# yahoo/CaffeOnSpark

Hardware: NVIDIA H100
Metric: images/sec (higher is better)
Workload: dtype f32

## Files before the change

### caffeonspark_b200/csrc/caffe_layers.cu

```cuda
#include <math.h>

#include "caffe_layers.hpp"

namespace cosb {
namespace {

struct FastDiv {
  unsigned d, m, s;
  explicit FastDiv(unsigned div) : d(div), m(0), s(0) {
    while (s < 31 && (1u << s) < d) ++s;
    m = (unsigned)((((1ull << 32) * ((1ull << s) - d)) / d) + 1);
  }
  __device__ __forceinline__ unsigned div(unsigned n) const { return (__umulhi(n, m) + n) >> s; }
};

constexpr int kLrnChunk = 16;
constexpr int kLrnBlock = 128;

template <int HALF>
__global__ void __launch_bounds__(kLrnBlock) lrn_forward_kernel(const float* __restrict__ x, float* __restrict__ y,
                                                                int C, FastDiv fd_hw, unsigned npix, int nchunks,
                                                                float alpha_over_n, float beta, float k) {
  const int chunk = blockIdx.x % nchunks;
  const unsigned p = (blockIdx.x / nchunks) * kLrnBlock + threadIdx.x;
  if (p >= npix) return;
  const unsigned HW = fd_hw.d, n = fd_hw.div(p);
  const size_t base = (size_t)n * C * HW + (p - n * HW);
  const int c0 = chunk * kLrnChunk;
  float xv[kLrnChunk + 2 * HALF];
#pragma unroll
  for (int i = 0; i < kLrnChunk + 2 * HALF; ++i) {
    const int c = c0 - HALF + i;
    xv[i] = (c >= 0 && c < C) ? x[base + (size_t)c * HW] : 0.f;
  }
#pragma unroll
  for (int t = 0; t < kLrnChunk; ++t) {
    const int c = c0 + t;
    if (c < C) {
      float ss = 0.f;
#pragma unroll
      for (int j = 0; j <= 2 * HALF; ++j) ss += xv[t + j] * xv[t + j];
      const float s = k + alpha_over_n * ss;
      y[base + (size_t)c * HW] = xv[t + HALF] * powf(s, -beta);
    }
  }
}

template <int HALF>
__global__ void __launch_bounds__(kLrnBlock) lrn_backward_kernel(const float* __restrict__ x,
                                                                 const float* __restrict__ dy, float* __restrict__ dx,
                                                                 int C, FastDiv fd_hw, unsigned npix, int nchunks,
                                                                 float alpha_over_n, float beta, float k, float coef) {
  const int chunk = blockIdx.x % nchunks;
  const unsigned p = (blockIdx.x / nchunks) * kLrnBlock + threadIdx.x;
  if (p >= npix) return;
  const unsigned HW = fd_hw.d, n = fd_hw.div(p);
  const size_t base = (size_t)n * C * HW + (p - n * HW);
  const int c0 = chunk * kLrnChunk;
  constexpr int NR = kLrnChunk + 2 * HALF;
  float xv[NR + 2 * HALF];
  float dv[NR];
#pragma unroll
  for (int i = 0; i < NR + 2 * HALF; ++i) {
    const int c = c0 - 2 * HALF + i;
    xv[i] = (c >= 0 && c < C) ? x[base + (size_t)c * HW] : 0.f;
  }
#pragma unroll
  for (int i = 0; i < NR; ++i) {
    const int c = c0 - HALF + i;
    dv[i] = (c >= 0 && c < C) ? dy[base + (size_t)c * HW] : 0.f;
  }
  float r[NR], sb[NR];
#pragma unroll
  for (int i = 0; i < NR; ++i) {
    const int c = c0 - HALF + i;
    float ss = 0.f;
#pragma unroll
    for (int j = 0; j <= 2 * HALF; ++j) ss += xv[i + j] * xv[i + j];
    const float s = k + alpha_over_n * ss;
    sb[i] = powf(s, -beta);
    r[i] = (c >= 0 && c < C) ? dv[i] * xv[i + HALF] * sb[i] / s : 0.f;
  }
#pragma unroll
  for (int t = 0; t < kLrnChunk; ++t) {
    const int c = c0 + t;
    if (c < C) {
      float acc = 0.f;
#pragma unroll
      for (int j = 0; j <= 2 * HALF; ++j) acc += r[t + j];
      dx[base + (size_t)c * HW] = dv[t + HALF] * sb[t + HALF] - coef * xv[t + 2 * HALF] * acc;
    }
  }
}

template <template <int> class Launch, typename... A>
cudaError_t lrn_dispatch(int half, A... args) {
  switch (half) {
    case 0: return Launch<0>::run(args...);
    case 1: return Launch<1>::run(args...);
    case 2: return Launch<2>::run(args...);
    case 3: return Launch<3>::run(args...);
    case 4: return Launch<4>::run(args...);
    case 5: return Launch<5>::run(args...);
    case 6: return Launch<6>::run(args...);
    case 7: return Launch<7>::run(args...);
  }
  return cudaErrorInvalidValue;
}

struct LrnGrid {
  long long npix;
  int nchunks;
  long long blocks;
  FastDiv fd_hw;
  LrnGrid(int num, int channels, int hw)
      : npix((long long)num * hw), nchunks((channels + kLrnChunk - 1) / kLrnChunk),
        blocks(((npix + kLrnBlock - 1) / kLrnBlock) * nchunks), fd_hw(hw) {}
  bool fits() const { return npix < (1ll << 31) && blocks < (1ll << 31); }
};

template <int HALF>
struct LrnFwd {
  static cudaError_t run(const float* x, float* y, int C, const LrnGrid& g, float aon, float beta, float k,
                         cudaStream_t st) {
    lrn_forward_kernel<HALF><<<(unsigned)g.blocks, kLrnBlock, 0, st>>>(x, y, C, g.fd_hw, (unsigned)g.npix,
                                                                        g.nchunks, aon, beta, k);
    return cudaGetLastError();
  }
};

template <int HALF>
struct LrnBwd {
  static cudaError_t run(const float* x, const float* dy, float* dx, int C, const LrnGrid& g, float aon, float beta,
                         float k, float coef, cudaStream_t st) {
    lrn_backward_kernel<HALF><<<(unsigned)g.blocks, kLrnBlock, 0, st>>>(x, dy, dx, C, g.fd_hw, (unsigned)g.npix,
                                                                         g.nchunks, aon, beta, k, coef);
    return cudaGetLastError();
  }
};


template <int KERNEL, int STRIDE>
__global__ void pool_forward_kernel(const float* __restrict__ x, const float* __restrict__ bias,
                                    float* __restrict__ y, uint8_t* __restrict__ index, unsigned total, FastDiv fd_pp,
                                    FastDiv fd_pw, FastDiv fd_c, int H, int W, int kernel_rt, int stride_rt) {
  const int kernel = KERNEL ? KERNEL : kernel_rt, stride = STRIDE ? STRIDE : stride_rt;
  const unsigned i = blockIdx.x * blockDim.x + threadIdx.x;
  if (i >= total) return;
  const unsigned plane = fd_pp.div(i);
  const unsigned e = i - plane * fd_pp.d;
  const int ph = (int)fd_pw.div(e);
  const int pw = (int)(e - ph * fd_pw.d);
  const float b = bias[plane - fd_c.div(plane) * fd_c.d];
  const float* xp = x + (size_t)plane * H * W;
  const int hs = ph * stride, ws = pw * stride;
  float vmax = -INFINITY;
  int pos = 0;
#pragma unroll
  for (int dh = 0; dh < (KERNEL ? KERNEL : 15); ++dh) {
    if (dh >= kernel || hs + dh >= H) break;
#pragma unroll
    for (int dw = 0; dw < (KERNEL ? KERNEL : 15); ++dw) {
      if (dw >= kernel || ws + dw >= W) break;
      const float v = xp[(hs + dh) * W + ws + dw] + b;
      if (v > vmax || isnan(v)) {
        vmax = v;
        pos = dh * kernel + dw;
      }
    }
  }
  const bool pass = vmax > 0.f || isnan(vmax);
  y[i] = pass ? vmax : 0.f;
  index[i] = pass ? (uint8_t)pos : kPoolNoGrad;
}

template <int KERNEL, int STRIDE>
__global__ void pool_backward_kernel(const float* __restrict__ dy, const uint8_t* __restrict__ index,
                                     float* __restrict__ dx, float* __restrict__ partials, FastDiv fd_w, int H,
                                     int kernel_rt, int stride_rt, int PH, int PW) {
  const int kernel = KERNEL ? KERNEL : kernel_rt, stride = STRIDE ? STRIDE : stride_rt;
  const int W = (int)fd_w.d;
  const long long plane = blockIdx.x;
  const float* dyp = dy + (size_t)plane * PH * PW;
  const uint8_t* ip = index + (size_t)plane * PH * PW;
  float* dxp = dx + (size_t)plane * H * W;
  float part = 0.f;
  for (int e = threadIdx.x; e < H * W; e += blockDim.x) {
    const int h = (int)fd_w.div(e), w = e - h * W;
    const int phs = h < kernel ? 0 : (h - kernel) / stride + 1, phe = min(h / stride + 1, PH);
    const int pws = w < kernel ? 0 : (w - kernel) / stride + 1, pwe = min(w / stride + 1, PW);
    float g = 0.f;
    if (KERNEL) {
      constexpr int NW = KERNEL ? (KERNEL + STRIDE - 1) / STRIDE : 1;
      unsigned id[NW][NW];
      float v[NW][NW];
#pragma unroll
      for (int a = 0; a < NW; ++a) {
#pragma unroll
        for (int b = 0; b < NW; ++b) {
          const bool ok = phs + a < phe && pws + b < pwe;
          const int o = ok ? (phs + a) * PW + pws + b : 0;
          id[a][b] = ok ? ip[o] : kPoolNoGrad;
          v[a][b] = ok ? dyp[o] : 0.f;
        }
      }
#pragma unroll
      for (int a = 0; a < NW; ++a) {
#pragma unroll
        for (int b = 0; b < NW; ++b)
          g += id[a][b] == (unsigned)((h - (phs + a) * stride) * kernel + (w - (pws + b) * stride)) ? v[a][b] : 0.f;
      }
    } else {
      for (int ph = phs; ph < phe; ++ph) {
        for (int pw = pws; pw < pwe; ++pw) {
          if (ip[ph * PW + pw] == (h - ph * stride) * kernel + (w - pw * stride)) g += dyp[ph * PW + pw];
        }
      }
    }
    dxp[e] = g;
    part += g;
  }
  __shared__ float warp_sums[32];
#pragma unroll
  for (int o = 16; o > 0; o >>= 1) part += __shfl_xor_sync(0xffffffffu, part, o);
  if ((threadIdx.x & 31) == 0) warp_sums[threadIdx.x >> 5] = part;
  __syncthreads();
  if (threadIdx.x == 0) {
    float s = 0.f;
    for (int i = 0; i < (int)(blockDim.x >> 5); ++i) s += warp_sums[i];
    partials[plane] = s;
  }
}

__global__ void bias_grad_kernel(const float* __restrict__ partials, float* __restrict__ dbias, int N, int C) {
  const int c = blockIdx.x * blockDim.x + threadIdx.x;
  if (c >= C) return;
  float s = 0.f;
  for (int n = 0; n < N; ++n) s += partials[(size_t)n * C + c];
  dbias[c] = s;
}

}

cudaError_t lrn_forward(const float* x, float* y, int num, int channels, int height, int width, int local_size,
                        float alpha, float beta, float k, cudaStream_t stream) {
  const LrnGrid g(num, channels, height * width);
  if (g.blocks == 0) return cudaSuccess;
  if (!g.fits()) return cudaErrorInvalidValue;
  return lrn_dispatch<LrnFwd>(local_size / 2, x, y, channels, g, alpha / local_size, beta, k, stream);
}

cudaError_t lrn_backward(const float* x, const float* dy, float* dx, int num, int channels, int height, int width,
                         int local_size, float alpha, float beta, float k, cudaStream_t stream) {
  const LrnGrid g(num, channels, height * width);
  if (g.blocks == 0) return cudaSuccess;
  if (!g.fits()) return cudaErrorInvalidValue;
  return lrn_dispatch<LrnBwd>(local_size / 2, x, dy, dx, channels, g, alpha / local_size, beta, k,
                              2.f * alpha * beta / local_size, stream);
}

int pooled_size(int in, int kernel, int stride) {
  if (kernel < 1 || stride < 1 || in < kernel) return -1;
  int out = (in - kernel + stride - 1) / stride + 1;
  if ((out - 1) * stride >= in) --out;
  return out;
}

cudaError_t bias_relu_maxpool_forward(const float* x, const float* bias, float* y, uint8_t* index, int num,
                                      int channels, int height, int width, int kernel, int stride, int pooled_h,
                                      int pooled_w, cudaStream_t stream) {
  const long long total = (long long)num * channels * pooled_h * pooled_w;
  if (total == 0) return cudaSuccess;
  if (total >= (1ll << 31) || (long long)height * width >= (1ll << 31)) return cudaErrorInvalidValue;
  const int block = 256;
  const unsigned grid = (unsigned)((total + block - 1) / block);
  const FastDiv fpp(pooled_h * pooled_w), fpw(pooled_w), fc(channels);
  if (kernel == 3 && stride == 2)
    pool_forward_kernel<3, 2><<<grid, block, 0, stream>>>(x, bias, y, index, (unsigned)total, fpp, fpw, fc, height,
                                                          width, kernel, stride);
  else
    pool_forward_kernel<0, 0><<<grid, block, 0, stream>>>(x, bias, y, index, (unsigned)total, fpp, fpw, fc, height,
                                                          width, kernel, stride);
  return cudaGetLastError();
}

cudaError_t bias_relu_maxpool_backward(const float* dy, const uint8_t* index, float* dx, float* dbias_partials,
                                       float* dbias, int num, int channels, int height, int width, int kernel,
                                       int stride, int pooled_h, int pooled_w, cudaStream_t stream) {
  const long long planes = (long long)num * channels;
  if (channels == 0) return cudaSuccess;
  if (planes > 0) {
    if (planes >= (1ll << 31) || (long long)height * width >= (1ll << 31)) return cudaErrorInvalidValue;
    const int hw = height * width;
    const int block = hw >= 256 ? 256 : ((hw + 31) / 32) * 32;
    const FastDiv fw(width);
    if (kernel == 3 && stride == 2)
      pool_backward_kernel<3, 2><<<(unsigned)planes, block, 0, stream>>>(dy, index, dx, dbias_partials, fw, height,
                                                                         kernel, stride, pooled_h, pooled_w);
    else
      pool_backward_kernel<0, 0><<<(unsigned)planes, block, 0, stream>>>(dy, index, dx, dbias_partials, fw, height,
                                                                         kernel, stride, pooled_h, pooled_w);
    cudaError_t e = cudaGetLastError();
    if (e != cudaSuccess) return e;
  }
  bias_grad_kernel<<<(channels + 127) / 128, 128, 0, stream>>>(dbias_partials, dbias, num, channels);
  return cudaGetLastError();
}

}
```

Before: 19560.

## Tile LRN backward through shared memory and add 2x2-tiled k3s2 pool backward

The LRN backward kernel becomes a 2D block of 32 pixels by 8 channel rows with 32-channel chunks staged in shared memory. This shrinks the halo re-read fraction and the per-thread register arrays, at the cost of two block syncs. The max-pool backward for kernel 3, stride 2 gets a dedicated kernel in which each thread handles a 2x2 output tile and loads the 4 covering pooled entries once, sharing index and gradient loads across the tile. The block-sum reduction is factored into a helper.

```diff
diff --git a/caffeonspark_b200/csrc/caffe_layers.cu b/caffeonspark_b200/csrc/caffe_layers.cu
--- a/caffeonspark_b200/csrc/caffe_layers.cu
+++ b/caffeonspark_b200/csrc/caffe_layers.cu
@@ -46,49 +46,57 @@
   }
 }
 
+constexpr int kLrnBwdPix = 32;
+constexpr int kLrnBwdRows = 8;
+constexpr int kLrnBwdChunk = 32;
+
 template <int HALF>
-__global__ void __launch_bounds__(kLrnBlock) lrn_backward_kernel(const float* __restrict__ x,
-                                                                 const float* __restrict__ dy, float* __restrict__ dx,
-                                                                 int C, FastDiv fd_hw, unsigned npix, int nchunks,
-                                                                 float alpha_over_n, float beta, float k, float coef) {
+__global__ void __launch_bounds__(kLrnBwdPix* kLrnBwdRows)
+    lrn_backward_kernel(const float* __restrict__ x, const float* __restrict__ dy, float* __restrict__ dx, int C,
+                        FastDiv fd_hw, unsigned npix, int nchunks, float alpha_over_n, float beta, float k,
+                        float coef) {
+  constexpr int NX = kLrnBwdChunk + 4 * HALF;
+  constexpr int NR = kLrnBwdChunk + 2 * HALF;
+  __shared__ float sx[NX][kLrnBwdPix], sd[NR][kLrnBwdPix], sr[NR][kLrnBwdPix], ssb[kLrnBwdChunk][kLrnBwdPix];
+  const int tx = threadIdx.x, ty = threadIdx.y;
   const int chunk = blockIdx.x % nchunks;
-  const unsigned p = (blockIdx.x / nchunks) * kLrnBlock + threadIdx.x;
-  if (p >= npix) return;
-  const unsigned HW = fd_hw.d, n = fd_hw.div(p);
-  const size_t base = (size_t)n * C * HW + (p - n * HW);
-  const int c0 = chunk * kLrnChunk;
-  constexpr int NR = kLrnChunk + 2 * HALF;
-  float xv[NR + 2 * HALF];
-  float dv[NR];
-#pragma unroll
-  for (int i = 0; i < NR + 2 * HALF; ++i) {
+  const unsigned p = (blockIdx.x / nchunks) * kLrnBwdPix + tx;
+  const bool live = p < npix;
+  const unsigned HW = fd_hw.d, n = live ? fd_hw.div(p) : 0;
+  const size_t base = live ? (size_t)n * C * HW + (p - n * HW) : 0;
+  const int c0 = chunk * kLrnBwdChunk;
+#pragma unroll
+  for (int i = ty; i < NX; i += kLrnBwdRows) {
     const int c = c0 - 2 * HALF + i;
-    xv[i] = (c >= 0 && c < C) ? x[base + (size_t)c * HW] : 0.f;
-  }
-#pragma unroll
-  for (int i = 0; i < NR; ++i) {
+    sx[i][tx] = (live && c >= 0 && c < C) ? x[base + (size_t)c * HW] : 0.f;
+  }
+#pragma unroll
+  for (int i = ty; i < NR; i += kLrnBwdRows) {
     const int c = c0 - HALF + i;
-    dv[i] = (c >= 0 && c < C) ? dy[base + (size_t)c * HW] : 0.f;
-  }
-  float r[NR], sb[NR];
-#pragma unroll
-  for (int i = 0; i < NR; ++i) {
+    sd[i][tx] = (live && c >= 0 && c < C) ? dy[base + (size_t)c * HW] : 0.f;
+  }
+  __syncthreads();
+#pragma unroll
+  for (int i = ty; i < NR; i += kLrnBwdRows) {
     const int c = c0 - HALF + i;
     float ss = 0.f;
 #pragma unroll
-    for (int j = 0; j <= 2 * HALF; ++j) ss += xv[i + j] * xv[i + j];
+    for (int j = 0; j <= 2 * HALF; ++j) ss += sx[i + j][tx] * sx[i + j][tx];
     const float s = k + alpha_over_n * ss;
-    sb[i] = powf(s, -beta);
-    r[i] = (c >= 0 && c < C) ? dv[i] * xv[i + HALF] * sb[i] / s : 0.f;
-  }
-#pragma unroll
-  for (int t = 0; t < kLrnChunk; ++t) {
+    const float sb = powf(s, -beta);
+    sr[i][tx] = (c >= 0 && c < C) ? sd[i][tx] * sx[i + HALF][tx] * sb / s : 0.f;
+    if (i >= HALF && i < HALF + kLrnBwdChunk) ssb[i - HALF][tx] = sb;
+  }
+  __syncthreads();
+  if (!live) return;
+#pragma unroll
+  for (int t = ty; t < kLrnBwdChunk; t += kLrnBwdRows) {
     const int c = c0 + t;
     if (c < C) {
       float acc = 0.f;
 #pragma unroll
-      for (int j = 0; j <= 2 * HALF; ++j) acc += r[t + j];
-      dx[base + (size_t)c * HW] = dv[t + HALF] * sb[t + HALF] - coef * xv[t + 2 * HALF] * acc;
+      for (int j = 0; j <= 2 * HALF; ++j) acc += sr[t + j][tx];
+      dx[base + (size_t)c * HW] = sd[t + HALF][tx] * ssb[t][tx] - coef * sx[t + 2 * HALF][tx] * acc;
     }
   }
 }
@@ -113,9 +121,9 @@
   int nchunks;
   long long blocks;
   FastDiv fd_hw;
-  LrnGrid(int num, int channels, int hw)
-      : npix((long long)num * hw), nchunks((channels + kLrnChunk - 1) / kLrnChunk),
-        blocks(((npix + kLrnBlock - 1) / kLrnBlock) * nchunks), fd_hw(hw) {}
+  LrnGrid(int num, int channels, int hw, int chunk, int pix)
+      : npix((long long)num * hw), nchunks((channels + chunk - 1) / chunk),
+        blocks(((npix + pix - 1) / pix) * nchunks), fd_hw(hw) {}
   bool fits() const { return npix < (1ll << 31) && blocks < (1ll << 31); }
 };
 
@@ -133,8 +141,8 @@
 struct LrnBwd {
   static cudaError_t run(const float* x, const float* dy, float* dx, int C, const LrnGrid& g, float aon, float beta,
                          float k, float coef, cudaStream_t st) {
-    lrn_backward_kernel<HALF><<<(unsigned)g.blocks, kLrnBlock, 0, st>>>(x, dy, dx, C, g.fd_hw, (unsigned)g.npix,
-                                                                         g.nchunks, aon, beta, k, coef);
+    lrn_backward_kernel<HALF><<<(unsigned)g.blocks, dim3(kLrnBwdPix, kLrnBwdRows), 0, st>>>(
+        x, dy, dx, C, g.fd_hw, (unsigned)g.npix, g.nchunks, aon, beta, k, coef);
     return cudaGetLastError();
   }
 };
@@ -174,11 +182,22 @@
   index[i] = pass ? (uint8_t)pos : kPoolNoGrad;
 }
 
-template <int KERNEL, int STRIDE>
+__device__ __forceinline__ void store_block_sum(float part, float* out) {
+  __shared__ float warp_sums[32];
+#pragma unroll
+  for (int o = 16; o > 0; o >>= 1) part += __shfl_xor_sync(0xffffffffu, part, o);
+  if ((threadIdx.x & 31) == 0) warp_sums[threadIdx.x >> 5] = part;
+  __syncthreads();
+  if (threadIdx.x == 0) {
+    float s = 0.f;
+    for (int i = 0; i < (int)(blockDim.x >> 5); ++i) s += warp_sums[i];
+    *out = s;
+  }
+}
+
 __global__ void pool_backward_kernel(const float* __restrict__ dy, const uint8_t* __restrict__ index,
                                      float* __restrict__ dx, float* __restrict__ partials, FastDiv fd_w, int H,
-                                     int kernel_rt, int stride_rt, int PH, int PW) {
-  const int kernel = KERNEL ? KERNEL : kernel_rt, stride = STRIDE ? STRIDE : stride_rt;
+                                     int kernel, int stride, int PH, int PW) {
   const int W = (int)fd_w.d;
   const long long plane = blockIdx.x;
   const float* dyp = dy + (size_t)plane * PH * PW;
@@ -190,46 +209,62 @@
     const int phs = h < kernel ? 0 : (h - kernel) / stride + 1, phe = min(h / stride + 1, PH);
     const int pws = w < kernel ? 0 : (w - kernel) / stride + 1, pwe = min(w / stride + 1, PW);
     float g = 0.f;
-    if (KERNEL) {
-      constexpr int NW = KERNEL ? (KERNEL + STRIDE - 1) / STRIDE : 1;
-      unsigned id[NW][NW];
-      float v[NW][NW];
-#pragma unroll
-      for (int a = 0; a < NW; ++a) {
-#pragma unroll
-        for (int b = 0; b < NW; ++b) {
-          const bool ok = phs + a < phe && pws + b < pwe;
-          const int o = ok ? (phs + a) * PW + pws + b : 0;
-          id[a][b] = ok ? ip[o] : kPoolNoGrad;
-          v[a][b] = ok ? dyp[o] : 0.f;
-        }
-      }
-#pragma unroll
-      for (int a = 0; a < NW; ++a) {
-#pragma unroll
-        for (int b = 0; b < NW; ++b)
-          g += id[a][b] == (unsigned)((h - (phs + a) * stride) * kernel + (w - (pws + b) * stride)) ? v[a][b] : 0.f;
-      }
-    } else {
-      for (int ph = phs; ph < phe; ++ph) {
-        for (int pw = pws; pw < pwe; ++pw) {
-          if (ip[ph * PW + pw] == (h - ph * stride) * kernel + (w - pw * stride)) g += dyp[ph * PW + pw];
-        }
+    for (int ph = phs; ph < phe; ++ph) {
+      for (int pw = pws; pw < pwe; ++pw) {
+        if (ip[ph * PW + pw] == (h - ph * stride) * kernel + (w - pw * stride)) g += dyp[ph * PW + pw];
       }
     }
     dxp[e] = g;
     part += g;
   }
-  __shared__ float warp_sums[32];
-#pragma unroll
-  for (int o = 16; o > 0; o >>= 1) part += __shfl_xor_sync(0xffffffffu, part, o);
-  if ((threadIdx.x & 31) == 0) warp_sums[threadIdx.x >> 5] = part;
-  __syncthreads();
-  if (threadIdx.x == 0) {
-    float s = 0.f;
-    for (int i = 0; i < (int)(blockDim.x >> 5); ++i) s += warp_sums[i];
-    partials[plane] = s;
-  }
+  store_block_sum(part, partials + plane);
+}
+
+__global__ void pool_backward_k3s2_kernel(const float* __restrict__ dy, const uint8_t* __restrict__ index,
+                                          float* __restrict__ dx, float* __restrict__ partials, FastDiv fd_tq, int H,
+                                          int W, int PH, int PW) {
+  const long long plane = blockIdx.x;
+  const float* dyp = dy + (size_t)plane * PH * PW;
+  const uint8_t* ip = index + (size_t)plane * PH * PW;
+  float* dxp = dx + (size_t)plane * H * W;
+  const int TQ = (int)fd_tq.d, tiles = ((H + 1) / 2) * TQ;
+  float part = 0.f;
+  for (int e = threadIdx.x; e < tiles; e += blockDim.x) {
+    const int p = (int)fd_tq.div(e), q = e - p * TQ;
+    unsigned id[2][2];
+    float v[2][2];
+#pragma unroll
+    for (int a = 0; a < 2; ++a) {
+#pragma unroll
+      for (int b = 0; b < 2; ++b) {
+        const int ph = p - 1 + a, pw = q - 1 + b;
+        const bool ok = ph >= 0 && ph < PH && pw >= 0 && pw < PW;
+        const int o = ok ? ph * PW + pw : 0;
+        id[a][b] = ok ? ip[o] : kPoolNoGrad;
+        v[a][b] = ok ? dyp[o] : 0.f;
+      }
+    }
+#pragma unroll
+    for (int r = 0; r < 2; ++r) {
+#pragma unroll
+      for (int c = 0; c < 2; ++c) {
+        const int h = 2 * p + r, w = 2 * q + c;
+        if (h >= H || w >= W) continue;
+        float g = 0.f;
+#pragma unroll
+        for (int a = 0; a < 2; ++a) {
+#pragma unroll
+          for (int b = 0; b < 2; ++b) {
+            const int dh = 2 + r - 2 * a, dw = 2 + c - 2 * b;
+            if (dh <= 2 && dw <= 2) g += id[a][b] == (unsigned)(dh * 3 + dw) ? v[a][b] : 0.f;
+          }
+        }
+        dxp[h * W + w] = g;
+        part += g;
+      }
+    }
+  }
+  store_block_sum(part, partials + plane);
 }
 
 __global__ void bias_grad_kernel(const float* __restrict__ partials, float* __restrict__ dbias, int N, int C) {
@@ -244,7 +279,7 @@
 
 cudaError_t lrn_forward(const float* x, float* y, int num, int channels, int height, int width, int local_size,
                         float alpha, float beta, float k, cudaStream_t stream) {
-  const LrnGrid g(num, channels, height * width);
+  const LrnGrid g(num, channels, height * width, kLrnChunk, kLrnBlock);
   if (g.blocks == 0) return cudaSuccess;
   if (!g.fits()) return cudaErrorInvalidValue;
   return lrn_dispatch<LrnFwd>(local_size / 2, x, y, channels, g, alpha / local_size, beta, k, stream);
@@ -252,7 +287,7 @@
 
 cudaError_t lrn_backward(const float* x, const float* dy, float* dx, int num, int channels, int height, int width,
                          int local_size, float alpha, float beta, float k, cudaStream_t stream) {
-  const LrnGrid g(num, channels, height * width);
+  const LrnGrid g(num, channels, height * width, kLrnBwdChunk, kLrnBwdPix);
   if (g.blocks == 0) return cudaSuccess;
   if (!g.fits()) return cudaErrorInvalidValue;
   return lrn_dispatch<LrnBwd>(local_size / 2, x, dy, dx, channels, g, alpha / local_size, beta, k,
@@ -291,15 +326,15 @@
   if (channels == 0) return cudaSuccess;
   if (planes > 0) {
     if (planes >= (1ll << 31) || (long long)height * width >= (1ll << 31)) return cudaErrorInvalidValue;
-    const int hw = height * width;
-    const int block = hw >= 256 ? 256 : ((hw + 31) / 32) * 32;
-    const FastDiv fw(width);
-    if (kernel == 3 && stride == 2)
-      pool_backward_kernel<3, 2><<<(unsigned)planes, block, 0, stream>>>(dy, index, dx, dbias_partials, fw, height,
-                                                                         kernel, stride, pooled_h, pooled_w);
+    const bool k3s2 = kernel == 3 && stride == 2;
+    const int work = k3s2 ? ((height + 1) / 2) * ((width + 1) / 2) : height * width;
+    const int block = work >= 256 ? 256 : ((work + 31) / 32) * 32;
+    if (k3s2)
+      pool_backward_k3s2_kernel<<<(unsigned)planes, block, 0, stream>>>(
+          dy, index, dx, dbias_partials, FastDiv((width + 1) / 2), height, width, pooled_h, pooled_w);
     else
-      pool_backward_kernel<0, 0><<<(unsigned)planes, block, 0, stream>>>(dy, index, dx, dbias_partials, fw, height,
-                                                                         kernel, stride, pooled_h, pooled_w);
+      pool_backward_kernel<<<(unsigned)planes, block, 0, stream>>>(dy, index, dx, dbias_partials, FastDiv(width),
+                                                                   height, kernel, stride, pooled_h, pooled_w);
     cudaError_t e = cudaGetLastError();
     if (e != cudaSuccess) return e;
   }
```

Measured after the change: 20120, median of 6. 2.8% higher.
